# tskare/gpuaudiobench

Measured on AMD Instinct MI355X. Metric: audio_buffers_per_sec, higher is better.
Workload: dtype f32

## Files before the change

### gpuaudiobench_amd/csrc/k_conv_accel.hip

```cpp
#include <hip/hip_runtime.h>
#include <hip/hip_ext.h>

#include <cmath>
#include <cstdlib>
#include <algorithm>
#include <chrono>
#include <mutex>
#include <string>
#include <thread>
#include <type_traits>
#include <utility>
#include <vector>

#include "gab_common.hpp"
#include "gab_fft.hpp"
#include "k_conv_fdl.hpp"

namespace gab {
namespace fft {

void build_twiddles(float* t) {
    for (int m = 0; m < kTwiddleN; ++m) {
        double a = -2.0 * M_PI * (double)m / (double)kTwiddleN;
        t[2 * m] = (float)std::cos(a);
        t[2 * m + 1] = (float)std::sin(a);
    }
}

const cf* device_twiddles() {
    static std::mutex mu;
    static std::vector<cf*> per_device(64, nullptr);
    int dev = 0;
    GAB_HIP_CHECK(hipGetDevice(&dev));
    std::lock_guard<std::mutex> lock(mu);
    if (dev >= (int)per_device.size()) per_device.resize(dev + 1, nullptr);
    if (!per_device[dev]) {
        std::vector<float> host(2 * kTwiddleN);
        build_twiddles(host.data());
        cf* d = nullptr;
        GAB_HIP_CHECK(hipMalloc(&d, sizeof(cf) * kTwiddleN));
        GAB_HIP_CHECK(hipMemcpy(d, host.data(), sizeof(cf) * kTwiddleN, hipMemcpyHostToDevice));
        per_device[dev] = d;
    }
    return per_device[dev];
}

}

using fft::cf;
using fft::mk;

namespace {

constexpr int kB = 512;
constexpr int kNA = 1024;
constexpr int kNB = 4096;
constexpr int kSlots = 8;
constexpr int kBinsA = kNA / 2 + 1;
constexpr int kBinsB = kNB / 2 + 1;
constexpr int kThreads = 256;

using PadB = fft::Pad<16>;
constexpr int kLdsHalf = PadB::size(kNB);

using fft::partner_exchange;

template <int N, int R>
__device__ __forceinline__ void load_spectra(float4 (&c)[R], const float4* __restrict__ pm, int tid) {
    constexpr int NT = N / R;
#pragma unroll
    for (int r = 0; r < R; ++r) {
        const int k = tid + r * NT;
        if (r < R / 2) c[r] = pm[k];
        else if (r > R / 2) c[r] = pm[N - k];
        else c[r] = pm[tid == 0 ? k : N - k];
    }
}

template <int N, int R>
__device__ __forceinline__ void spectral_product(cf (&z)[R], const cf (&zraw)[R], const float4 (&c)[R],
                                                 int tid) {
#pragma unroll
    for (int r = 0; r < R; ++r) {
        cf P = mk(c[r].x, c[r].y), M = mk(c[r].z, c[r].w);
        if (r > R / 2 || (r == R / 2 && tid != 0)) {
            z[r] = fft::cfma_cjcj(zraw[r], M, fft::cmulc(z[r], P));
        } else {
            z[r] = fft::cfma_cj(zraw[r], M, fft::cmul(z[r], P));
        }
    }
}

template <bool STREAM, bool TAIL, bool LOOPED = false>
__device__ __forceinline__ void conv_one_buffer(
    const float* __restrict__ in, float* __restrict__ out, float* __restrict__ hist,
    const float4* __restrict__ pmA, const float4* __restrict__ pmB,
    const cf* __restrict__ tw, int T, int head, cf* __restrict__ lds) {
    cf* const lds0 = lds;
    cf* const lds1 = lds + kLdsHalf;
// ... 500 lines not shown
    unsigned* const gw = rt.counters + 32 * g;
    if (tid == 0) {
        const unsigned old = __hip_atomic_fetch_add(&gw[0], 1u, __ATOMIC_RELAXED, __HIP_MEMORY_SCOPE_AGENT);
        int role = 1;
        if (old + 1u == rt.epoch * (unsigned)members) {
            role = 2;
            __hip_atomic_store(&gw[1], 0u, __ATOMIC_RELAXED, __HIP_MEMORY_SCOPE_AGENT);
            asm volatile("s_waitcnt vmcnt(0)" ::: "memory");
            __hip_atomic_store(&gw[2], rt.epoch, __ATOMIC_RELAXED, __HIP_MEMORY_SCOPE_AGENT);
        } else {
            int tries = 0;
            while (__hip_atomic_load(&gw[2], __ATOMIC_RELAXED, __HIP_MEMORY_SCOPE_AGENT) != rt.epoch) {
                if (++tries > (1 << 10)) { role = 0; break; }
                __builtin_amdgcn_s_sleep(3);
            }
        }
        s_word = role;
    }
    __syncthreads();
    const int role = s_word;
    if (role == 0) return;
    const int row_f4 = members / 2;
    const auto srd = __builtin_amdgcn_make_buffer_rsrc(rt.park, 0, (int)((size_t)T * kB * 4), 0x00020000);
    const int col0 = 2 * first;
    unsigned drained = 0;
    for (;;) {
        __syncthreads();
        if (tid == 0) s_word = (int)__hip_atomic_fetch_add(&gw[1], 1u, __ATOMIC_RELAXED, __HIP_MEMORY_SCOPE_AGENT);
        __syncthreads();
        const int share = s_word;
        if (share >= members) break;
        const int i = share * kThreads + tid;
        const int sidx = i / row_f4, c = i - sidx * row_f4;
        const auto raw = __builtin_amdgcn_raw_buffer_load_b128(srd, 4u * (unsigned)(T * sidx + col0 + 4 * c), 0, 16);
        typedef float f4v __attribute__((ext_vector_type(4)));
        const f4v val = {__uint_as_float(raw[0]), __uint_as_float(raw[1]), __uint_as_float(raw[2]), __uint_as_float(raw[3])};
        float* const dst = rt.h_out + (size_t)T * sidx + col0 + 4 * c;
        asm volatile("global_store_dwordx4 %0, %1, off sc0 sc1" ::"v"(dst), "v"(val) : "memory");
        ++drained;
        if (role != 2) break;
    }
    asm volatile("s_waitcnt vmcnt(0)" ::: "memory");
    __syncthreads();
    GAB_RT_STAMP_MAX(g, 3);
    if (tid == 0 && drained) {
        const unsigned old = __hip_atomic_fetch_add(&rt.counters[32 * rt.groups], drained, __ATOMIC_RELAXED, __HIP_MEMORY_SCOPE_AGENT);
        if (old + drained == rt.epoch * (unsigned)gridDim.x) {
            __hip_atomic_store(rt.done, rt.epoch, __ATOMIC_RELAXED, __HIP_MEMORY_SCOPE_SYSTEM);
            GAB_RT_STAMP_MAX(64, 0);
        }
    }
}

__global__ __launch_bounds__(kThreads, 2) void conv_batch_kernel(
    const float* __restrict__ in, float* __restrict__ out, float* __restrict__ hist,
    const float4* __restrict__ pmA, const float4* __restrict__ pmB,
    const cf* __restrict__ tw, int T, int head, int n_buffers) {
    __shared__ cf lds[2 * kLdsHalf];
    const size_t step = (size_t)T * kB;
    for (int nb = 0; nb < n_buffers; ++nb)
        conv_one_buffer<true, true, true>(in + nb * step, out + nb * step, hist, pmA, pmB, tw, T,
                                             (head + nb) & (kSlots - 1), lds);
}

constexpr int kBatchBarriers = 6;

struct ConvEngine {
    const unsigned* doorbell;
    unsigned* relay;
    unsigned* progress;
    unsigned* completed;
    unsigned* error;
    int ring;
    int poll_every_period;
    unsigned* started;
    unsigned* resident;
    unsigned long long idle_ticks;
};
constexpr double kEngineIdleSeconds = 4.0;

typedef unsigned u4 __attribute__((ext_vector_type(4)));

constexpr int kB12Threads = 768;
constexpr int kB12SpecCf = 4 * kBinsA * 2;
constexpr int kB12Tw1Cf = 16 * 15;
constexpr int kB12Lds = 6 * kWaveImg + 2 * kLdsHalf + kB12SpecCf + kB12Tw1Cf;

template <int N, int R, int R0, int R1, class PM>
__device__ __forceinline__ void load_spectra_part(float4 (&c)[R1 - R0], PM pm, int tid) {
    constexpr int NT = N / R;
#pragma unroll
    for (int r = R0; r < R1; ++r) {
        const int k = tid + r * NT;
        if (r < R / 2) c[r - R0] = pm[k];
        else if (r > R / 2) c[r - R0] = pm[N - k];
        else c[r - R0] = pm[tid == 0 ? k : N - k];
    }
}
template <int N, int R, int R0, int R1>
__device__ __forceinline__ void spectral_product_part(cf (&z)[R], const cf (&zraw)[R1 - R0], const float4 (&c)[R1 - R0], int tid) {
#pragma unroll
    for (int r = R0; r < R1; ++r) {
        cf P = mk(c[r - R0].x, c[r - R0].y), M = mk(c[r - R0].z, c[r - R0].w);
        if (r > R / 2 || (r == R / 2 && tid != 0)) z[r] = fft::cfma_cjcj(zraw[r - R0], M, fft::cmulc(z[r], P));
        else z[r] = fft::cfma_cj(zraw[r - R0], M, fft::cmul(z[r], P));
    }
}

#ifdef GAB_ABLATE
__device__ unsigned long long g_split_stamps[2 * 8 * 8192];
#define GAB_B12BAR(period, i)                                                                                         \
    do {                                                                                                              \
        if ((sp.debug & 64) && ((period) == 32 || (period) == 33) && lane == 0)                                       \
            g_split_stamps[(((size_t)blockIdx.x * 12 + w) * 2 + ((period) - 32)) * 6 + (i)] = __builtin_amdgcn_s_memrealtime(); \
        __syncthreads();                                                                                              \
    } while (0)
#else
#define GAB_B12BAR(period, i) __syncthreads()
#endif
__device__ __forceinline__ void conv_split_batch12_resident(
    const float* __restrict__ in, float* __restrict__ out, float* __restrict__ hist,
    const float4* __restrict__ pmA, const ConvSplit& sp, const cf* __restrict__ tw, int T, int head0, int n_buffers,
    cf* __restrict__ lds) {
    cf* const far_img = lds + 6 * kWaveImg;
    float4* const spec = reinterpret_cast<float4*>(far_img + 2 * kLdsHalf);
    cf* const tw1 = reinterpret_cast<cf*>(spec + 4 * kBinsA);
    const int tid = threadIdx.x;
    const int d = xcd_contiguous(blockIdx.x, gridDim.x);
    const size_t step = (size_t)T * kB;
    {
        const float4* const gA = pmA + (size_t)(2 * d) * kBinsA;
        const float4* const gA2 = sp.pmA2 + (size_t)(2 * d) * kBinsA;
        for (int i = tid; i < 2 * kBinsA; i += kB12Threads) { spec[i] = gA[i]; spec[2 * kBinsA + i] = gA2[i]; }
        if (tid < 16) {
            cf pw[15];
            fft::powers_of<16>(tw[tid * (fft::kTwiddleN / 256)], pw);
#pragma unroll
            for (int r = 0; r < 15; ++r) tw1[tid * 15 + r] = pw[r];
        }
    }
    __syncthreads();
    const int lane = tid & 63;
    const int w = __builtin_amdgcn_readfirstlane(tid >> 6);
    const unsigned rb = (unsigned)lane + ((unsigned)lane >> 4);
    auto in_slot = [&](int slot) -> const float* { return in + (size_t)slot * step; };
    auto idle_period = [&]() { for (int i = 0; i < kBatchBarriers; ++i) __syncthreads(); };

    if (w >= 4) {
        const int g = __builtin_amdgcn_readfirstlane((w - 4) >> 2);
        const int ft = (tid - kThreads) & (kThreads - 1);
        cf* const img = far_img + g * kLdsHalf;
        const int q = 2 * d + g;
        const cf* const hp = reinterpret_cast<const cf*>(hist) + (size_t)q * kSlots * kB;
        cf* const cg = sp.carry + (size_t)q * kCarrySlots * kB;
        const size_t ca = (size_t)(2 * q) * kB, cb_ = ca + kB;
        const float4* const pf = sp.pmF + (size_t)q * kBinsB;
        using B16 = fft::Butterfly<16, false>;
        using B16i = fft::Butterfly<16, true>;
        cf tw2[15];
        fft::powers_of<16>(tw[ft], tw2);
        auto opaque_t = [&]() -> unsigned { unsigned v = (unsigned)ft; asm volatile("" : "+v"(v)); return v; };
        auto w0_of = [](unsigned t) -> unsigned { return t * 17u; };
        auto rd_of = [](unsigned t) -> unsigned { return t + (t >> 4); };
        auto w1_of = [](unsigned t) -> unsigned { const unsigned b1 = (t >> 4) * 256u + (t & 15u); return b1 + (b1 >> 4); };
        auto tw1row_of = [&](unsigned t) -> const cf* { return tw1 + (t & 15u) * 15u; };
        auto load_window = [&](auto part_tag, int nb, cf (&z)[16]) {
            constexpr int PART = decltype(part_tag)::value;
            const int head = (head0 + nb) & (kSlots - 1);
            int fo = ft;
            asm volatile("" : "+v"(fo));
            if constexpr (PART == 0) {
                const float* const cur = in_slot(nb);
                z[14] = mk(cur[ca + fo], cur[cb_ + fo]);
                z[15] = mk(cur[ca + fo + kThreads], cur[cb_ + fo + kThreads]);
            }
            constexpr int BL0 = PART == 0 ? 4 : 0, BL1 = PART == 0 ? 7 : 4;
            if (nb >= kSlots - 1) {
#pragma unroll
                for (int bl = BL0; bl < BL1; ++bl) {
                    const float* const src = in_slot(nb - (7 - bl));
                    z[2 * bl] = mk(src[ca + fo], src[cb_ + fo]);
                    z[2 * bl + 1] = mk(src[ca + fo + kThreads], src[cb_ + fo + kThreads]);
                }
            } else {
#pragma unroll
                for (int bl = BL0; bl < BL1; ++bl) {
                    if (nb - 7 + bl >= 0) {
                        const float* const src = in_slot(nb - (7 - bl));
                        z[2 * bl] = mk(src[ca + fo], src[cb_ + fo]);
                        z[2 * bl + 1] = mk(src[ca + fo + kThreads], src[cb_ + fo + kThreads]);
                    } else {
                        const int s = ((head + 1 + bl) & (kSlots - 1)) * kB;
                        z[2 * bl] = hp[s + fo];
                        z[2 * bl + 1] = hp[s + kThreads + fo];
                    }
                }
            }
        };
        cf z[16], zn[16];
        auto first_half = [&](int nb) {
#pragma unroll
            for (int r = 0; r < 16; ++r) z[r] = zn[r];
            B16::run(z);
            {
                const unsigned w0 = w0_of(opaque_t());
#pragma unroll
                for (int r = 0; r < 16; ++r) img[w0 + r] = z[B16::out_slot(r)];
            }
            GAB_B12BAR(nb, 0);
            {
                const unsigned t = opaque_t(), rd = rd_of(t);
                const cf* const tw1row = tw1row_of(t);
#pragma unroll
                for (int r = 0; r < 16; ++r) z[r] = img[rd + 272 * r];
#pragma unroll
                for (int r = 1; r < 16; ++r) z[r] = fft::cmul(z[r], tw1row[r - 1]);
            }
            B16::run(z);
            GAB_B12BAR(nb, 1);
            {
                const unsigned w1 = w1_of(opaque_t());
#pragma unroll
                for (int r = 0; r < 16; ++r) img[w1 + 17 * r] = z[B16::out_slot(r)];
            }
            __builtin_amdgcn_sched_barrier(0);
            float4 clo[8], chi[8];
            {
                int fo = ft;
                asm volatile("" : "+v"(fo));
                load_spectra_part<kNB, 16, 0, 8>(clo, pf, fo);
            }
            __builtin_amdgcn_sched_barrier(0);
            GAB_B12BAR(nb, 2);
            {
                const unsigned rd = rd_of(opaque_t());
#pragma unroll
                for (int r = 0; r < 16; ++r) z[r] = img[rd + 272 * r];
            }
#pragma unroll
            for (int r = 1; r < 16; ++r) z[r] = fft::cmul(z[r], tw2[r - 1]);
            __builtin_amdgcn_sched_barrier(0);
            {
                int fo = ft;
                asm volatile("" : "+v"(fo));
                load_spectra_part<kNB, 16, 8, 16>(chi, pf, fo);
            }
            __builtin_amdgcn_sched_barrier(0);
            B16::run(z);
            GAB_B12BAR(nb, 3);
            {
                const unsigned t = opaque_t();
#pragma unroll
                for (int r = 0; r < 16; ++r) img[t + 256u * r] = z[B16::out_slot(r)];
            }
            GAB_B12BAR(nb, 4);
            {
                cf o[16];
#pragma unroll
                for (int r = 0; r < 16; ++r) o[r] = z[B16::out_slot(r)];
#pragma unroll
                for (int r = 0; r < 16; ++r) z[r] = o[r];
                const unsigned t = opaque_t();
                const cf* const pb = img + (kNB - 256 * 15) - t;
                cf zp[8];
                zp[0] = img[(kNB - t) & (kNB - 1)];
#pragma unroll
                for (int r = 1; r < 8; ++r) zp[r] = pb[256 * (15 - r)];
                spectral_product_part<kNB, 16, 0, 8>(z, zp, clo, ft);
#pragma unroll
                for (int r = 0; r < 8; ++r) zp[r] = pb[256 * (7 - r)];
                spectral_product_part<kNB, 16, 8, 16>(z, zp, chi, ft);
            }
            B16i::run(z);
            GAB_B12BAR(nb, 5);
        };
        auto second_half = [&](int period, int nb_done, int nb_next) {
            if (nb_next >= 0) {
                load_window(std::integral_constant<int, 0>{}, nb_next, zn);
            } else {
#pragma unroll
                for (int r = 0; r < 16; ++r) zn[r] = mk(0.0f, 0.0f);
            }
            GAB_B12BAR(period, 0);
            if (nb_done >= 0) {
                const unsigned w0 = w0_of(opaque_t());
#pragma unroll
                for (int r = 0; r < 16; ++r) img[w0 + r] = z[B16i::out_slot(r)];
            }
            GAB_B12BAR(period, 1);
            if (nb_done >= 0) {
                const unsigned t = opaque_t(), rd = rd_of(t);
                const cf* const tw1row = tw1row_of(t);
#pragma unroll
                for (int r = 0; r < 16; ++r) z[r] = img[rd + 272 * r];
#pragma unroll
                for (int r = 1; r < 16; ++r) z[r] = fft::cmulc(z[r], tw1row[r - 1]);
                B16i::run(z);
            }
            GAB_B12BAR(period, 2);
            if (nb_done >= 0) {
                const unsigned w1 = w1_of(opaque_t());
#pragma unroll
                for (int r = 0; r < 16; ++r) img[w1 + 17 * r] = z[B16i::out_slot(r)];
            }
            __builtin_amdgcn_sched_barrier(0);
            if (nb_next >= 0) load_window(std::integral_constant<int, 1>{}, nb_next, zn);
            __builtin_amdgcn_sched_barrier(0);
            GAB_B12BAR(period, 3);
            if (nb_done >= 0) {
                const unsigned rd = rd_of(opaque_t());
#pragma unroll
                for (int r = 0; r < 16; ++r) z[r] = img[rd + 272 * r];
#pragma unroll
                for (int r = 1; r < 16; ++r) z[r] = fft::cmulc(z[r], tw2[r - 1]);
                cf x12, x13, x14, x15;
                B16i::run_last4(z, x12, x13, x14, x15);
                const int head = (head0 + nb_done) & (kSlots - 1);
                cf* const c1 = cg + ((head + 1) & (kCarrySlots - 1)) * kB;
                cf* const c2 = cg + ((head + 2) & (kCarrySlots - 1)) * kB;
                c1[ft] = x12;
                c1[ft + kThreads] = x13;
                c2[ft] = x14;
                c2[ft + kThreads] = x15;
            }
            GAB_B12BAR(period, 4);
            if (nb_done >= 0) asm volatile("s_waitcnt vmcnt(0)" ::: "memory");
            GAB_B12BAR(period, 5);
        };
        const int first = (g - head0) & 1;
        int nb = 0;
        if (first == 1) {
            second_half(0, -1, 1 < n_buffers ? 1 : -1);
            nb = 1;
        } else if (n_buffers > 0) {
            load_window(std::integral_constant<int, 0>{}, 0, zn);
            load_window(std::integral_constant<int, 1>{}, 0, zn);
        }
        for (;;) {
            if (nb > n_buffers) break;
            if (nb < n_buffers) first_half(nb); else idle_period();
            ++nb;
            if (nb > n_buffers) break;
            second_half(nb, nb - 1 < n_buffers ? nb - 1 : -1, nb + 1 < n_buffers ? nb + 1 : -1);
            ++nb;
        }
    } else if (w < 2) {
        const int q = 2 * d + w;
        cf* const hp = reinterpret_cast<cf*>(hist) + (size_t)q * kSlots * kB;
        cf* const img = lds + w * kWaveImg;
        cf* const hand = lds + (2 + w) * kWaveImg;
        const float4* const sa = spec + w * kBinsA;
        const float4* const sa2 = spec + (2 + w) * kBinsA;
        using WF = fft::WaveFFT1024<false>;
        WF::Lean t;
        WF::load_twiddles(t, tw, lane);
        const size_t xoff = (size_t)(2 * q) * kB;
        cf z[16], prev[8], nxt[8];
        auto product_from_image = [&](cf (&v)[16], const float4* sp_lds) {
            {
                cf zp[8];
                float4 ch[8];
#pragma unroll
                for (int r = 0; r < 8; ++r) zp[r] = img[PadA16::at((kNA - (lane + 64 * r)) & (kNA - 1))];
                load_spectra_part<kNA, 16, 0, 8>(ch, sp_lds, lane);
                spectral_product_part<kNA, 16, 0, 8>(v, zp, ch, lane);
            }
            __builtin_amdgcn_sched_barrier(0);
            {
                cf zp[8];
                float4 ch[8];
#pragma unroll
                for (int r = 0; r < 8; ++r) zp[r] = img[PadA16::at((kNA - (lane + 64 * (8 + r))) & (kNA - 1))];
                load_spectra_part<kNA, 16, 8, 16>(ch, sp_lds, lane);
                spectral_product_part<kNA, 16, 8, 16>(v, zp, ch, lane);
            }
        };
        {
            const int s1 = ((head0 + kSlots - 1) & (kSlots - 1)) * kB, s2 = ((head0 + kSlots - 2) & (kSlots - 1)) * kB;
#pragma unroll
            for (int j = 0; j < 8; ++j) z[j] = hp[s2 + lane + 64 * j];
#pragma unroll
            for (int j = 0; j < 8; ++j) prev[j] = hp[s1 + lane + 64 * j];
            if (n_buffers > 0) {
                const float* const x0 = in_slot(0) + xoff;
#pragma unroll
                for (int j = 0; j < 8; ++j) nxt[j] = mk(x0[lane + 64 * j], x0[kB + lane + 64 * j]);
            }
#pragma unroll
            for (int j = 0; j < 8; ++j) z[8 + j] = prev[j];
            WF::run(z, img, t, lane, WF::NoHook());
#pragma unroll
            for (int r = 0; r < 16; ++r) img[rb + 68 * r] = z[r];
            __builtin_amdgcn_wave_barrier();
        }
        for (int nb = 0; nb < n_buffers; ++nb) {
            const int head = (head0 + nb) & (kSlots - 1);
            {
                cf share[16];
#pragma unroll
                for (int r = 0; r < 16; ++r) share[r] = img[rb + 68 * r];
                product_from_image(share, sa2);
                GAB_B12BAR(nb, 0);
#pragma unroll
                for (int r = 0; r < 16; ++r) hand[rb + 68 * r] = share[r];
            }
            __builtin_amdgcn_sched_barrier(0);
#pragma unroll
            for (int j = 0; j < 8; ++j) { z[j] = prev[j]; z[8 + j] = nxt[j]; }
            if (nb + kSlots >= n_buffers) {
#pragma unroll
                for (int j = 0; j < 8; ++j) hp[head * kB + lane + 64 * j] = nxt[j];
            }
#pragma unroll
            for (int j = 0; j < 8; ++j) prev[j] = nxt[j];
            if (nb + 1 < n_buffers) {
                int lo = lane;
                asm volatile("" : "+v"(lo));
                const float* const xa = in_slot(nb + 1) + xoff + lo;
#pragma unroll
                for (int j = 0; j < 8; ++j) nxt[j] = mk(xa[64 * j], xa[kB + 64 * j]);
            }
            WF::run(z, img, t, lane, [&](int i) { GAB_B12BAR(nb, 1 + i); });
            GAB_B12BAR(nb, 3);
#pragma unroll
            for (int r = 0; r < 16; ++r) img[rb + 68 * r] = z[r];
            __builtin_amdgcn_wave_barrier();
            product_from_image(z, sa);
            GAB_B12BAR(nb, 4);
#pragma unroll
            for (int r = 0; r < 16; ++r) hand[rb + 68 * r] = fft::cadd(z[r], hand[rb + 68 * r]);
            GAB_B12BAR(nb, 5);
        }
        idle_period();
    } else {
        const int pr = w - 2;
        const cf* const hand = lds + (2 + pr) * kWaveImg;
        cf* const img = lds + (4 + pr) * kWaveImg;
        const cf* const other = lds + (4 + (1 - pr)) * kWaveImg;
        const cf* const cg = sp.carry + (size_t)(2 * d + pr) * kCarrySlots * kB;
        using WFi = fft::WaveFFT1024<true>;
        WFi::Lean t;
        WFi::load_twiddles(t, tw, lane);
        idle_period();
        for (int nb = 1; nb <= n_buffers; ++nb) {
            const int b = nb - 1;
            const int head = (head0 + b) & (kSlots - 1);
            float* const outb = out + (size_t)b * step;
            cf z[16], y[8], park[8];
#pragma unroll
            for (int r = 0; r < 16; ++r) z[r] = hand[rb + 68 * r];
            {
                int lo = lane;
                asm volatile("" : "+v"(lo));
                const unsigned long long* const cy = reinterpret_cast<const unsigned long long*>(cg + (head & (kCarrySlots - 1)) * kB + lo);
#pragma unroll
                for (int j = 0; j < 8; ++j) {
                    const unsigned long long v = __hip_atomic_load(cy + 64 * j, __ATOMIC_RELAXED, __HIP_MEMORY_SCOPE_AGENT);
                    park[j] = mk(__uint_as_float((unsigned)v), __uint_as_float((unsigned)(v >> 32)));
                }
            }
            GAB_B12BAR(nb, 0);
            WFi::run(z, img, t, lane, [&](int i) { GAB_B12BAR(nb, 1 + i); });
#pragma unroll
            for (int j = 0; j < 8; ++j) y[j] = fft::cadd(z[8 + j], park[j]);
            GAB_B12BAR(nb, 3);
            if (pr == 0) {
#pragma unroll
                for (int j = 0; j < 4; ++j) img[lane + 64 * j] = y[4 + j];
            } else {
#pragma unroll
                for (int j = 0; j < 4; ++j) img[lane + 64 * j] = y[j];
            }
            GAB_B12BAR(nb, 4);
            {
                float* const o0 = outb + 4 * (size_t)d;
                if (pr == 0) {
#pragma unroll
                    for (int j = 0; j < 4; ++j) {
                        const cf theirs = other[lane + 64 * j];
                        *reinterpret_cast<float4*>(o0 + (size_t)T * (lane + 64 * j)) = make_float4(y[j].x, y[j].y, theirs.x, theirs.y);
                    }
                } else {
#pragma unroll
                    for (int j = 0; j < 4; ++j) {
                        const cf theirs = other[lane + 64 * j];
                        *reinterpret_cast<float4*>(o0 + (size_t)T * (lane + 64 * (4 + j))) = make_float4(theirs.x, theirs.y, y[4 + j].x, y[4 + j].y);
                    }
                }
            }
            GAB_B12BAR(nb, 5);
        }
    }
}

__global__ __launch_bounds__(kB12Threads) void conv_split_batch12_kernel(
    const float* __restrict__ in, float* __restrict__ out, float* __restrict__ hist,
    const float4* __restrict__ pmA, ConvSplit sp, const cf* __restrict__ tw, int T, int head0, int n_buffers) {
    __shared__ __attribute__((aligned(16))) cf lds[kB12Lds];
    conv_split_batch12_resident(in, out, hist, pmA, sp, tw, T, head0, n_buffers, lds);
}

#ifdef GAB_ABLATE
#define GAB_E12BAR(i)                                                                                                 \
    do {                                                                                                              \
        if ((sp.debug & 64) && (nb == 4000 || nb == 4001) && lane == 0)                                               \
            g_split_stamps[(((size_t)blockIdx.x * 12 + w) * 2 + (nb - 4000)) * 6 + (i)] = __builtin_amdgcn_s_memrealtime(); \
        __syncthreads();                                                                                              \
    } while (0)
#else
#define GAB_E12BAR(i) __syncthreads()
#endif
__device__ __forceinline__ void conv_split_engine12_resident(
    const float* __restrict__ in, float* __restrict__ out, float* __restrict__ hist,
    const float4* __restrict__ pmA, const ConvSplit& sp, const cf* __restrict__ tw, int T, int head0,
    const ConvEngine& eng, cf* __restrict__ lds, unsigned* __restrict__ s_door) {
    constexpr bool ENGINE = true;
    constexpr int n_buffers = 0;
    (void)ENGINE; (void)n_buffers;
    cf* const far_img = lds + 6 * kWaveImg;
    float4* const spec = reinterpret_cast<float4*>(far_img + 2 * kLdsHalf);
    cf* const tw1 = reinterpret_cast<cf*>(spec + 4 * kBinsA);
    const int tid = threadIdx.x;
    const int d = xcd_contiguous(blockIdx.x, gridDim.x);
    const size_t step = (size_t)T * kB;
    {
        const float4* const gA = pmA + (size_t)(2 * d) * kBinsA;
        const float4* const gA2 = sp.pmA2 + (size_t)(2 * d) * kBinsA;
        for (int i = tid; i < 2 * kBinsA; i += kB12Threads) { spec[i] = gA[i]; spec[2 * kBinsA + i] = gA2[i]; }
        if (tid < 16) {
            cf pw[15];
            fft::powers_of<16>(tw[tid * (fft::kTwiddleN / 256)], pw);
#pragma unroll
            for (int r = 0; r < 15; ++r) tw1[tid * 15 + r] = pw[r];
        }
    }
    constexpr int kPoller = 2 * 64;
    auto read_door = [&]() -> unsigned {
        if (blockIdx.x == 0) {
            const unsigned v = __hip_atomic_load(eng.doorbell, __ATOMIC_RELAXED, __HIP_MEMORY_SCOPE_SYSTEM);
            __hip_atomic_store(eng.relay, v, __ATOMIC_RELAXED, __HIP_MEMORY_SCOPE_AGENT);
            return v;
        }
        return __hip_atomic_load(eng.relay, __ATOMIC_RELAXED, __HIP_MEMORY_SCOPE_AGENT);
    };
    if (tid == 0) {
        s_door[2] = 0;
        const unsigned before = __hip_atomic_fetch_add(eng.started, 1u, __ATOMIC_RELAXED, __HIP_MEMORY_SCOPE_AGENT);
        if (before == 0) __hip_atomic_store(&eng.resident[0], 1u, __ATOMIC_RELAXED, __HIP_MEMORY_SCOPE_SYSTEM);
        if (before + 1 == gridDim.x) __hip_atomic_store(&eng.resident[1], gridDim.x, __ATOMIC_RELAXED, __HIP_MEMORY_SCOPE_SYSTEM);
    }
    __syncthreads();
    const int lane = tid & 63;
    const int w = __builtin_amdgcn_readfirstlane(tid >> 6);
    const unsigned rb = (unsigned)lane + ((unsigned)lane >> 4);
    const bool aggregator = blockIdx.x == (gridDim.x > 1 ? 1u : 0u);
    unsigned reported = 0;
    auto aggregate_request = [&](u4& a, u4& b) {
        const auto srd = __builtin_amdgcn_make_buffer_rsrc(eng.progress, 0, (int)(8u * gridDim.x), 0x00020000);
        a = __builtin_amdgcn_raw_buffer_load_b128(srd, 32u * (unsigned)lane, 0, 16);
        b = __builtin_amdgcn_raw_buffer_load_b128(srd, 32u * (unsigned)lane + 16u, 0, 16);
    };
    auto aggregate_report = [&](const u4& a, const u4& b) {
        const unsigned words = 2u * gridDim.x;
        auto pick = [&](unsigned v, unsigned idx) { return idx < words ? v : 0xffffffffu; };
        unsigned m = min(min(min(pick(a[0], 8u * lane), pick(a[1], 8u * lane + 1)), min(pick(a[2], 8u * lane + 2), pick(a[3], 8u * lane + 3))),
                         min(min(pick(b[0], 8u * lane + 4), pick(b[1], 8u * lane + 5)), min(pick(b[2], 8u * lane + 6), pick(b[3], 8u * lane + 7))));
#pragma unroll
        for (int o = 32; o > 0; o >>= 1) m = min(m, (unsigned)__shfl_xor((int)m, o));
        if (m != reported) {
            reported = m;
            if (lane == 0) __hip_atomic_store(eng.completed, m, __ATOMIC_RELAXED, __HIP_MEMORY_SCOPE_SYSTEM);
        }
    };
    auto gate = [&](int nb, bool idle) -> int {
        {
            if (idle && __builtin_amdgcn_readfirstlane(s_door[2]) != 0) return -1;
            bool look = !idle;
            for (;;) {
                if (look) {
                    const unsigned D = __builtin_amdgcn_readfirstlane(s_door[nb & 1]);
                    const int pub = (int)(D & 0x3fffffffu);
                    const bool stop = (D >> 31) != 0, flush = ((D >> 30) & 1u) != 0;
                    if (pub >= nb + 2 || ((stop || flush) && pub >= nb + 1)) return pub;
                    if (stop) return -1;
                }
                look = true;
                __syncthreads();
                if (w == 2) {
                    unsigned v = 0;
                    int tries = 0;
                    const unsigned long long t_poll = __builtin_amdgcn_s_memrealtime();
                    for (;;) {
                        u4 pa, pb;
                        if (aggregator) aggregate_request(pa, pb);
                        unsigned mine = 0;
                        if (lane == 0) mine = read_door();
                        v = __builtin_amdgcn_readfirstlane(mine);
                        if (aggregator) aggregate_report(pa, pb);
                        const int p2 = (int)(v & 0x3fffffffu);
                        if (p2 >= nb + 2 || (v >> 31) || (((v >> 30) & 1u) && p2 >= nb + 1)) break;
                        if ((++tries & 255) == 0 && __builtin_amdgcn_s_memrealtime() - t_poll > eng.idle_ticks) {
                            if (lane == 0) {
                                __hip_atomic_store(eng.error, 1u, __ATOMIC_RELAXED, __HIP_MEMORY_SCOPE_SYSTEM);
                                s_door[2] = 1;
                            }
                            v = 0x80000000u | (unsigned)(p2 < nb ? p2 : nb);
                            break;
                        }
                        __builtin_amdgcn_s_sleep(6);
                    }
                    if (lane == 0) s_door[nb & 1] = v;
                }
                __syncthreads();
            }
        }
    };
    auto in_slot = [&](int slot) -> const float* { return in + (size_t)slot * step; };
    auto next_slot = [&](int slot) -> int { return (ENGINE && slot + 1 == eng.ring) ? 0 : slot + 1; };
    auto ld = [](const float* p) -> float {
        if constexpr (ENGINE)
            return __hip_atomic_load(p, __ATOMIC_RELAXED, __HIP_MEMORY_SCOPE_SYSTEM);
        else return *p;
    };

    auto idle_period = [&]() { for (int i = 0; i < kBatchBarriers; ++i) __syncthreads(); };

    if (w >= 4) {
        const int g = __builtin_amdgcn_readfirstlane((w - 4) >> 2);
        const int ft = (tid - kThreads) & (kThreads - 1);
        cf* const img = far_img + g * kLdsHalf;
        const int q = 2 * d + g;
        const cf* const hp = reinterpret_cast<const cf*>(hist) + (size_t)q * kSlots * kB;
        cf* const cg = sp.carry + (size_t)q * kCarrySlots * kB;
        const size_t ca = (size_t)(2 * q) * kB, cb_ = ca + kB;
        const float4* const pf = sp.pmF + (size_t)q * kBinsB;
        using B16 = fft::Butterfly<16, false>;
        using B16i = fft::Butterfly<16, true>;
        const cf tw2_base = tw[ft];
        auto tw2_of = [&](cf (&w)[15]) {
            cf b = tw2_base;
            asm volatile("" : "+v"(b.x), "+v"(b.y));
            fft::powers_of<16>(b, w);
        };
        auto opaque_t = [&]() -> unsigned { unsigned v = (unsigned)ft; asm volatile("" : "+v"(v)); return v; };
        auto w0_of = [](unsigned t) -> unsigned { return t * 17u; };
        auto rd_of = [](unsigned t) -> unsigned { return t + (t >> 4); };
        auto w1_of = [](unsigned t) -> unsigned { const unsigned b1 = (t >> 4) * 256u + (t & 15u); return b1 + (b1 >> 4); };
        auto tw1row_of = [&](unsigned t) -> const cf* { return tw1 + (t & 15u) * 15u; };
        auto load_window = [&](auto part_tag, auto first_tag, int nb, int slot, int slot_before, cf (&z)[16]) {
            constexpr int PART = decltype(part_tag)::value;
            constexpr bool FIRST = decltype(first_tag)::value;
            const int head = (head0 + nb) & (kSlots - 1);
            int fo = ft;
            asm volatile("" : "+v"(fo));
            if constexpr (PART == 0) {
                const float* const cur = in_slot(slot);
                z[14] = mk(ld(cur + ca + fo), ld(cur + cb_ + fo));
                z[15] = mk(ld(cur + ca + fo + kThreads), ld(cur + cb_ + fo + kThreads));
                if constexpr (!FIRST) {
                    const float* const prv = in_slot(slot_before);
                    z[12] = mk(ld(prv + ca + fo), ld(prv + cb_ + fo));
                    z[13] = mk(ld(prv + ca + fo + kThreads), ld(prv + cb_ + fo + kThreads));
                } else {
                    const int s6 = ((head + kSlots - 1) & (kSlots - 1)) * kB;
                    z[12] = hp[s6 + fo];
                    z[13] = hp[s6 + kThreads + fo];
                }
#pragma unroll
                for (int bl = 4; bl < 6; ++bl) {
                    const int sb = ((head + 1 + bl) & (kSlots - 1)) * kB;
                    z[2 * bl] = hp[sb + fo];
                    z[2 * bl + 1] = hp[sb + kThreads + fo];
                }
            } else {
#pragma unroll
                for (int bl = 0; bl < 4; ++bl) {
                    const int sb = ((head + 1 + bl) & (kSlots - 1)) * kB;
                    z[2 * bl] = hp[sb + fo];
                    z[2 * bl + 1] = hp[sb + kThreads + fo];
                }
            }
        };
        cf z[16], zn[16];
        auto first_half = [&](int nb) {
#pragma unroll
            for (int r = 0; r < 16; ++r) z[r] = zn[r];
            B16::run(z);
            {
                const unsigned w0 = w0_of(opaque_t());
#pragma unroll
                for (int r = 0; r < 16; ++r) img[w0 + r] = z[B16::out_slot(r)];
            }
            GAB_E12BAR(0);
            {
                const unsigned t = opaque_t(), rd = rd_of(t);
                const cf* const tw1row = tw1row_of(t);
#pragma unroll
                for (int r = 0; r < 16; ++r) z[r] = img[rd + 272 * r];
#pragma unroll
                for (int r = 1; r < 16; ++r) z[r] = fft::cmul(z[r], tw1row[r - 1]);
            }
            B16::run(z);
            GAB_E12BAR(1);
            {
                const unsigned w1 = w1_of(opaque_t());
#pragma unroll
                for (int r = 0; r < 16; ++r) img[w1 + 17 * r] = z[B16::out_slot(r)];
            }
            __builtin_amdgcn_sched_barrier(0);
            float4 clo[8], chi[8];
            {
                int fo = ft;
                asm volatile("" : "+v"(fo));
                load_spectra_part<kNB, 16, 0, 8>(clo, pf, fo);
            }
            __builtin_amdgcn_sched_barrier(0);
            GAB_E12BAR(2);
            {
                const unsigned rd = rd_of(opaque_t());
#pragma unroll
                for (int r = 0; r < 16; ++r) z[r] = img[rd + 272 * r];
            }
            {
                cf tw2[15];
                tw2_of(tw2);
#pragma unroll
                for (int r = 1; r < 16; ++r) z[r] = fft::cmul(z[r], tw2[r - 1]);
            }
            __builtin_amdgcn_sched_barrier(0);
            {
                int fo = ft;
                asm volatile("" : "+v"(fo));
                load_spectra_part<kNB, 16, 8, 16>(chi, pf, fo);
            }
            __builtin_amdgcn_sched_barrier(0);
            B16::run(z);
            GAB_E12BAR(3);
            {
                const unsigned t = opaque_t();
#pragma unroll
                for (int r = 0; r < 16; ++r) img[t + 256u * r] = z[B16::out_slot(r)];
            }
            GAB_E12BAR(4);
            {
                cf o[16];
#pragma unroll
                for (int r = 0; r < 16; ++r) o[r] = z[B16::out_slot(r)];
#pragma unroll
                for (int r = 0; r < 16; ++r) z[r] = o[r];
                const unsigned t = opaque_t();
                const cf* const pb = img + (kNB - 256 * 15) - t;
                cf zp[8];
                zp[0] = img[(kNB - t) & (kNB - 1)];
#pragma unroll
                for (int r = 1; r < 8; ++r) zp[r] = pb[256 * (15 - r)];
                spectral_product_part<kNB, 16, 0, 8>(z, zp, clo, ft);
#pragma unroll
                for (int r = 0; r < 8; ++r) zp[r] = pb[256 * (7 - r)];
                spectral_product_part<kNB, 16, 8, 16>(z, zp, chi, ft);
            }
            B16i::run(z);
            GAB_E12BAR(5);
        };
        auto second_half = [&](int period, int nb_done, int nb_next, int slot_next, int slot_now) {
            const int nb = period;
            (void)nb;
            if (nb_next >= 0) {
                load_window(std::integral_constant<int, 0>{}, std::false_type{}, nb_next, slot_next, slot_now, zn);
            } else {
#pragma unroll
                for (int r = 0; r < 16; ++r) zn[r] = mk(0.0f, 0.0f);
            }
            GAB_E12BAR(0);
            if (nb_done >= 0) {
                const unsigned w0 = w0_of(opaque_t());
#pragma unroll
                for (int r = 0; r < 16; ++r) img[w0 + r] = z[B16i::out_slot(r)];
            }
            GAB_E12BAR(1);
            if (nb_done >= 0) {
                const unsigned t = opaque_t(), rd = rd_of(t);
                const cf* const tw1row = tw1row_of(t);
#pragma unroll
                for (int r = 0; r < 16; ++r) z[r] = img[rd + 272 * r];
#pragma unroll
                for (int r = 1; r < 16; ++r) z[r] = fft::cmulc(z[r], tw1row[r - 1]);
                B16i::run(z);
            }
            GAB_E12BAR(2);
            if (nb_done >= 0) {
                const unsigned w1 = w1_of(opaque_t());
#pragma unroll
                for (int r = 0; r < 16; ++r) img[w1 + 17 * r] = z[B16i::out_slot(r)];
            }
            __builtin_amdgcn_sched_barrier(0);
            if (nb_next >= 0) load_window(std::integral_constant<int, 1>{}, std::false_type{}, nb_next, slot_next, slot_now, zn);
            __builtin_amdgcn_sched_barrier(0);
            GAB_E12BAR(3);
            if (nb_done >= 0) {
                const unsigned rd = rd_of(opaque_t());
#pragma unroll
                for (int r = 0; r < 16; ++r) z[r] = img[rd + 272 * r];
                {
                    cf tw2[15];
                    tw2_of(tw2);
#pragma unroll
                    for (int r = 1; r < 16; ++r) z[r] = fft::cmulc(z[r], tw2[r - 1]);
                }
                cf x12, x13, x14, x15;
                B16i::run_last4(z, x12, x13, x14, x15);
                const int head = (head0 + nb_done) & (kSlots - 1);
                cf* const c1 = cg + ((head + 1) & (kCarrySlots - 1)) * kB;
                cf* const c2 = cg + ((head + 2) & (kCarrySlots - 1)) * kB;
                c1[ft] = x12;
                c1[ft + kThreads] = x13;
                c2[ft] = x14;
                c2[ft + kThreads] = x15;
            }
            GAB_E12BAR(4);
            if (nb_done >= 0) asm volatile("s_waitcnt vmcnt(0)" ::: "memory");
            GAB_E12BAR(5);
        };
        bool in_flight = false, have_window = false;
        int nb = 0, slot = 0;
        for (;;) {
            int avail = gate(nb, true);
            if (nb >= avail) break;
            for (;;) {
                const bool mine = ((head0 + nb) & 1) == g;
                if (mine) {
                    if (!have_window) {
                        load_window(std::integral_constant<int, 0>{}, std::true_type{}, nb, slot, 0, zn);
                        load_window(std::integral_constant<int, 1>{}, std::true_type{}, nb, slot, 0, zn);
                    }
                    first_half(nb);
                    in_flight = true;
                    have_window = false;
                } else {
                    const bool can = nb + 1 < avail;
                    second_half(nb, in_flight ? nb - 1 : -1, can ? nb + 1 : -1, next_slot(slot), slot);
                    have_window = can;
                    in_flight = false;
// ... 1573 lines not shown
```

Baseline: 207,500.

## Exchange far-FFT conjugate partner bins via permlane32 swap instead of LDS

Remaps the far-segment thread-to-column assignment so that each lane's conjugate-mirror column sits in the opposite half of the same wave. The spectral product can then fetch partner bins with permlane32_swap instead of writing the whole FFT image to LDS and reading it back. Columns 0 and 128 get special handling in wave 0. This removes an LDS store/load round trip per period, but the two barrier calls are kept, and the change adds cross-lane permute instructions and a remapping that has to be correct.

```diff
diff --git a/gpuaudiobench_amd/csrc/k_conv_accel.hip b/gpuaudiobench_amd/csrc/k_conv_accel.hip
--- a/gpuaudiobench_amd/csrc/k_conv_accel.hip
+++ b/gpuaudiobench_amd/csrc/k_conv_accel.hip
@@ -696,13 +696,71 @@
         else c[r - R0] = pm[tid == 0 ? k : N - k];
     }
 }
+template <int R>
+__device__ __forceinline__ void spectral_product_bin(cf& z, cf zraw, float4 c, int r, int tid) {
+    cf P = mk(c.x, c.y), M = mk(c.z, c.w);
+    if (r > R / 2 || (r == R / 2 && tid != 0)) z = fft::cfma_cjcj(zraw, M, fft::cmulc(z, P));
+    else z = fft::cfma_cj(zraw, M, fft::cmul(z, P));
+}
 template <int N, int R, int R0, int R1>
 __device__ __forceinline__ void spectral_product_part(cf (&z)[R], const cf (&zraw)[R1 - R0], const float4 (&c)[R1 - R0], int tid) {
 #pragma unroll
-    for (int r = R0; r < R1; ++r) {
-        cf P = mk(c[r - R0].x, c[r - R0].y), M = mk(c[r - R0].z, c[r - R0].w);
-        if (r > R / 2 || (r == R / 2 && tid != 0)) z[r] = fft::cfma_cjcj(zraw[r - R0], M, fft::cmulc(z[r], P));
-        else z[r] = fft::cfma_cj(zraw[r - R0], M, fft::cmul(z[r], P));
+    for (int r = R0; r < R1; ++r) spectral_product_bin<R>(z[r], zraw[r - R0], c[r - R0], r, tid);
+}
+
+__device__ __forceinline__ int far_column(int fw, int lane) {
+    const int c = lane < 32 ? 32 * fw + lane : 256 - 32 * fw - (lane - 32);
+    return c == 256 ? 128 : c;
+}
+__device__ __forceinline__ void half_swap(float& u, float& v) {
+    const auto a = __builtin_amdgcn_permlane32_swap(__float_as_uint(u), __float_as_uint(v), false, false);
+    const auto b = __builtin_amdgcn_permlane32_swap(a[1], a[0], false, false);
+    u = __uint_as_float(b[0]);
+    v = __uint_as_float(b[1]);
+}
+__device__ __forceinline__ void half_swap(cf& u, cf& v) {
+    float ux = u.x, uy = u.y, vx = v.x, vy = v.y;
+    half_swap(ux, vx);
+    half_swap(uy, vy);
+    u = mk(ux, uy);
+    v = mk(vx, vy);
+}
+__device__ __forceinline__ void far_partner_product(cf (&z)[16], const float4 (&clo)[8], const float4 (&chi)[8],
+                                                    int col, bool wave0, int lane) {
+    constexpr int G = 2;
+    cf raw[16];
+#pragma unroll
+    for (int r = 0; r < 16; ++r) raw[r] = z[r];
+#pragma unroll
+    for (int h = 0; h < 8 / G; ++h) {
+        cf pa[G], pb[G];
+#pragma unroll
+        for (int j = 0; j < G; ++j) {
+            const int r = G * h + j;
+            pa[j] = raw[15 - r];
+            pb[j] = raw[r];
+            half_swap(pa[j], pb[j]);
+        }
+        if (wave0) {
+            asm volatile("" ::: "memory");
+            if ((lane & 31) == 0) {
+                asm volatile("" ::: "memory");
+                const bool c0 = lane == 0;
+#pragma unroll
+                for (int j = 0; j < G; ++j) {
+                    const int r = G * h + j;
+                    pa[j] = c0 ? raw[(16 - r) & 15] : raw[15 - r];
+                    pb[j] = c0 ? raw[(r + 1) & 15] : raw[r];
+                }
+            }
+        }
+#pragma unroll
+        for (int j = 0; j < G; ++j) {
+            const int r = G * h + j;
+            spectral_product_bin<16>(z[r], pa[j], clo[r], r, col);
+            spectral_product_bin<16>(z[15 - r], pb[j], chi[7 - r], 15 - r, col);
+        }
+        __builtin_amdgcn_sched_barrier(0);
     }
 }
 
@@ -747,7 +805,8 @@
 
     if (w >= 4) {
         const int g = __builtin_amdgcn_readfirstlane((w - 4) >> 2);
-        const int ft = (tid - kThreads) & (kThreads - 1);
+        const bool fw0 = ((w - 4) & 3) == 0;
+        const int ft = far_column((w - 4) & 3, lane);
         cf* const img = far_img + g * kLdsHalf;
         const int q = 2 * d + g;
         const cf* const hp = reinterpret_cast<const cf*>(hist) + (size_t)q * kSlots * kB;
@@ -847,11 +906,6 @@
             __builtin_amdgcn_sched_barrier(0);
             B16::run(z);
             GAB_B12BAR(nb, 3);
-            {
-                const unsigned t = opaque_t();
-#pragma unroll
-                for (int r = 0; r < 16; ++r) img[t + 256u * r] = z[B16::out_slot(r)];
-            }
             GAB_B12BAR(nb, 4);
             {
                 cf o[16];
@@ -859,16 +913,7 @@
                 for (int r = 0; r < 16; ++r) o[r] = z[B16::out_slot(r)];
 #pragma unroll
                 for (int r = 0; r < 16; ++r) z[r] = o[r];
-                const unsigned t = opaque_t();
-                const cf* const pb = img + (kNB - 256 * 15) - t;
-                cf zp[8];
-                zp[0] = img[(kNB - t) & (kNB - 1)];
-#pragma unroll
-                for (int r = 1; r < 8; ++r) zp[r] = pb[256 * (15 - r)];
-                spectral_product_part<kNB, 16, 0, 8>(z, zp, clo, ft);
-#pragma unroll
-                for (int r = 0; r < 8; ++r) zp[r] = pb[256 * (7 - r)];
-                spectral_product_part<kNB, 16, 8, 16>(z, zp, chi, ft);
+                far_partner_product(z, clo, chi, ft, fw0, lane);
             }
             B16i::run(z);
             GAB_B12BAR(nb, 5);
@@ -1226,7 +1271,8 @@
 
     if (w >= 4) {
         const int g = __builtin_amdgcn_readfirstlane((w - 4) >> 2);
-        const int ft = (tid - kThreads) & (kThreads - 1);
+        const bool fw0 = ((w - 4) & 3) == 0;
+        const int ft = far_column((w - 4) & 3, lane);
         cf* const img = far_img + g * kLdsHalf;
         const int q = 2 * d + g;
         const cf* const hp = reinterpret_cast<const cf*>(hist) + (size_t)q * kSlots * kB;
@@ -1335,11 +1381,6 @@
             __builtin_amdgcn_sched_barrier(0);
             B16::run(z);
             GAB_E12BAR(3);
-            {
-                const unsigned t = opaque_t();
-#pragma unroll
-                for (int r = 0; r < 16; ++r) img[t + 256u * r] = z[B16::out_slot(r)];
-            }
             GAB_E12BAR(4);
             {
                 cf o[16];
@@ -1347,16 +1388,7 @@
                 for (int r = 0; r < 16; ++r) o[r] = z[B16::out_slot(r)];
 #pragma unroll
                 for (int r = 0; r < 16; ++r) z[r] = o[r];
-                const unsigned t = opaque_t();
-                const cf* const pb = img + (kNB - 256 * 15) - t;
-                cf zp[8];
-                zp[0] = img[(kNB - t) & (kNB - 1)];
-#pragma unroll
-                for (int r = 1; r < 8; ++r) zp[r] = pb[256 * (15 - r)];
-                spectral_product_part<kNB, 16, 0, 8>(z, zp, clo, ft);
-#pragma unroll
-                for (int r = 0; r < 8; ++r) zp[r] = pb[256 * (7 - r)];
-                spectral_product_part<kNB, 16, 8, 16>(z, zp, chi, ft);
+                far_partner_product(z, clo, chi, ft, fw0, lane);
             }
             B16i::run(z);
             GAB_E12BAR(5);
```

New measurement: 204,500. 1.5% lower.

## Restructure far-partition FFT LDS layout to cut per-period barriers from six to four

Applied to the files above, without the earlier changes.

Introduces a new LDS index layout for the far-tail 4096-point FFT in which the forward, spectral-product and inverse stages read and write each thread's values in place. This removes the separate write-back/read barrier pairs between passes. All wave roles in the batch12 kernel are re-synchronized to four barriers per period instead of six. The aim is less block-wide synchronization stall per audio buffer, at the cost of more intricate index arithmetic, a side slot for the Nyquist partner, and a higher risk of LDS bank conflicts or indexing errors.

```diff
diff --git a/gpuaudiobench_amd/csrc/k_conv_accel.hip b/gpuaudiobench_amd/csrc/k_conv_accel.hip
--- a/gpuaudiobench_amd/csrc/k_conv_accel.hip
+++ b/gpuaudiobench_amd/csrc/k_conv_accel.hip
@@ -15,6 +15,7 @@
 #include "gab_common.hpp"
 #include "gab_fft.hpp"
 #include "k_conv_fdl.hpp"
+#include "k_conv_far_layout.hpp"
 
 namespace gab {
 namespace fft {
@@ -681,6 +682,7 @@
 typedef unsigned u4 __attribute__((ext_vector_type(4)));
 
 constexpr int kB12Threads = 768;
+constexpr int kB12Barriers = 4;
 constexpr int kB12SpecCf = 4 * kBinsA * 2;
 constexpr int kB12Tw1Cf = 16 * 15;
 constexpr int kB12Lds = 6 * kWaveImg + 2 * kLdsHalf + kB12SpecCf + kB12Tw1Cf;
@@ -711,7 +713,7 @@
 #define GAB_B12BAR(period, i)                                                                                         \
     do {                                                                                                              \
         if ((sp.debug & 64) && ((period) == 32 || (period) == 33) && lane == 0)                                       \
-            g_split_stamps[(((size_t)blockIdx.x * 12 + w) * 2 + ((period) - 32)) * 6 + (i)] = __builtin_amdgcn_s_memrealtime(); \
+            g_split_stamps[(((size_t)blockIdx.x * 12 + w) * 2 + ((period) - 32)) * kB12Barriers + (i)] = __builtin_amdgcn_s_memrealtime(); \
         __syncthreads();                                                                                              \
     } while (0)
 #else
@@ -743,7 +745,7 @@
     const int w = __builtin_amdgcn_readfirstlane(tid >> 6);
     const unsigned rb = (unsigned)lane + ((unsigned)lane >> 4);
     auto in_slot = [&](int slot) -> const float* { return in + (size_t)slot * step; };
-    auto idle_period = [&]() { for (int i = 0; i < kBatchBarriers; ++i) __syncthreads(); };
+    auto idle_period = [&]() { for (int i = 0; i < kB12Barriers; ++i) __syncthreads(); };
 
     if (w >= 4) {
         const int g = __builtin_amdgcn_readfirstlane((w - 4) >> 2);
@@ -758,10 +760,8 @@
         using B16i = fft::Butterfly<16, true>;
         cf tw2[15];
         fft::powers_of<16>(tw[ft], tw2);
+        namespace FL = far_layout;
         auto opaque_t = [&]() -> unsigned { unsigned v = (unsigned)ft; asm volatile("" : "+v"(v)); return v; };
-        auto w0_of = [](unsigned t) -> unsigned { return t * 17u; };
-        auto rd_of = [](unsigned t) -> unsigned { return t + (t >> 4); };
-        auto w1_of = [](unsigned t) -> unsigned { const unsigned b1 = (t >> 4) * 256u + (t & 15u); return b1 + (b1 >> 4); };
         auto tw1row_of = [&](unsigned t) -> const cf* { return tw1 + (t & 15u) * 15u; };
         auto load_window = [&](auto part_tag, int nb, cf (&z)[16]) {
             constexpr int PART = decltype(part_tag)::value;
@@ -797,47 +797,58 @@
             }
         };
         cf z[16], zn[16];
-        auto first_half = [&](int nb) {
+        float4 clo[8], chi[8];
+        auto step_pass0 = [&]() {
 #pragma unroll
             for (int r = 0; r < 16; ++r) z[r] = zn[r];
             B16::run(z);
+            const unsigned t = opaque_t();
+#pragma unroll
+            for (int r = 0; r < 16; ++r) img[FL::pass0_write(t, r)] = z[B16::out_slot(r)];
+        };
+        auto step_pass1 = [&]() {
             {
-                const unsigned w0 = w0_of(opaque_t());
-#pragma unroll
-                for (int r = 0; r < 16; ++r) img[w0 + r] = z[B16::out_slot(r)];
-            }
-            GAB_B12BAR(nb, 0);
+                const unsigned t = opaque_t(), a = FL::a_base(t);
+                const cf* const tw1row = tw1row_of(t);
+#pragma unroll
+                for (int r = 0; r < 16; ++r) z[r] = img[a + 272 * r];
+#pragma unroll
+                for (int r = 1; r < 16; ++r) z[r] = fft::cmul(z[r], tw1row[r - 1]);
+            }
+            B16::run(z);
+            __builtin_amdgcn_sched_barrier(0);
             {
-                const unsigned t = opaque_t(), rd = rd_of(t);
-                const cf* const tw1row = tw1row_of(t);
-#pragma unroll
-                for (int r = 0; r < 16; ++r) z[r] = img[rd + 272 * r];
-#pragma unroll
-                for (int r = 1; r < 16; ++r) z[r] = fft::cmul(z[r], tw1row[r - 1]);
-            }
-            B16::run(z);
-            GAB_B12BAR(nb, 1);
-            {
-                const unsigned w1 = w1_of(opaque_t());
-#pragma unroll
-                for (int r = 0; r < 16; ++r) img[w1 + 17 * r] = z[B16::out_slot(r)];
+                const unsigned a = FL::a_base(opaque_t());
+#pragma unroll
+                for (int r = 0; r < 16; ++r) img[a + 272 * r] = z[B16::out_slot(r)];
             }
             __builtin_amdgcn_sched_barrier(0);
-            float4 clo[8], chi[8];
             {
                 int fo = ft;
                 asm volatile("" : "+v"(fo));
                 load_spectra_part<kNB, 16, 0, 8>(clo, pf, fo);
             }
             __builtin_amdgcn_sched_barrier(0);
-            GAB_B12BAR(nb, 2);
+        };
+        auto step_pass2 = [&]() {
             {
-                const unsigned rd = rd_of(opaque_t());
-#pragma unroll
-                for (int r = 0; r < 16; ++r) z[r] = img[rd + 272 * r];
+                const unsigned b = FL::pass2_base(opaque_t());
+#pragma unroll
+                for (int r = 0; r < 16; ++r) z[r] = img[b + 17 * r];
             }
 #pragma unroll
             for (int r = 1; r < 16; ++r) z[r] = fft::cmul(z[r], tw2[r - 1]);
+            B16::run(z);
+            __builtin_amdgcn_sched_barrier(0);
+            {
+                const unsigned t = opaque_t(), b = FL::pass2_base(t);
+#pragma unroll
+                for (int r = 0; r < 16; ++r) img[b + 17 * r] = z[B16::out_slot(r)];
+                if (t == 0) {
+#pragma unroll
+                    for (int r = 0; r < 16; ++r) img[FL::side_slot(r)] = z[B16::out_slot(r)];
+                }
+            }
             __builtin_amdgcn_sched_barrier(0);
             {
                 int fo = ft;
@@ -845,33 +856,78 @@
                 load_spectra_part<kNB, 16, 8, 16>(chi, pf, fo);
             }
             __builtin_amdgcn_sched_barrier(0);
-            B16::run(z);
-            GAB_B12BAR(nb, 3);
-            {
-                const unsigned t = opaque_t();
-#pragma unroll
-                for (int r = 0; r < 16; ++r) img[t + 256u * r] = z[B16::out_slot(r)];
-            }
-            GAB_B12BAR(nb, 4);
+        };
+        auto step_partner = [&]() {
             {
                 cf o[16];
 #pragma unroll
                 for (int r = 0; r < 16; ++r) o[r] = z[B16::out_slot(r)];
 #pragma unroll
                 for (int r = 0; r < 16; ++r) z[r] = o[r];
-                const unsigned t = opaque_t();
-                const cf* const pb = img + (kNB - 256 * 15) - t;
+                const cf* const pb = img + FL::partner_base(opaque_t());
                 cf zp[8];
-                zp[0] = img[(kNB - t) & (kNB - 1)];
-#pragma unroll
-                for (int r = 1; r < 8; ++r) zp[r] = pb[256 * (15 - r)];
+#pragma unroll
+                for (int r = 0; r < 8; ++r) zp[r] = pb[17 * (15 - r)];
                 spectral_product_part<kNB, 16, 0, 8>(z, zp, clo, ft);
 #pragma unroll
-                for (int r = 0; r < 8; ++r) zp[r] = pb[256 * (7 - r)];
+                for (int r = 0; r < 8; ++r) zp[r] = pb[17 * (7 - r)];
                 spectral_product_part<kNB, 16, 8, 16>(z, zp, chi, ft);
             }
             B16i::run(z);
-            GAB_B12BAR(nb, 5);
+            __builtin_amdgcn_sched_barrier(0);
+            {
+                cf* const pb = img + FL::partner_base(opaque_t());
+#pragma unroll
+                for (int r = 0; r < 16; ++r) pb[17 * r] = z[B16i::out_slot(r)];
+            }
+        };
+        auto step_inv1 = [&]() {
+            {
+                const unsigned t = opaque_t(), p0 = FL::inv1_first(t), pb = FL::inv1_base(t);
+                const cf* const tw1row = tw1row_of(t);
+                z[0] = img[p0];
+#pragma unroll
+                for (int r = 1; r < 16; ++r) z[r] = img[pb - 272 * r];
+#pragma unroll
+                for (int r = 1; r < 16; ++r) z[r] = fft::cmulc(z[r], tw1row[r - 1]);
+            }
+            B16i::run(z);
+            __builtin_amdgcn_sched_barrier(0);
+            {
+                const unsigned t = opaque_t(), p0 = FL::inv1_first(t), pb = FL::inv1_base(t);
+                img[p0] = z[B16i::out_slot(0)];
+#pragma unroll
+                for (int r = 1; r < 16; ++r) img[pb - 272 * r] = z[B16i::out_slot(r)];
+            }
+        };
+        auto step_inv2 = [&](int nb_done) {
+            {
+                const unsigned t = opaque_t(), p0 = FL::inv2_first(t), pb = FL::inv2_base(t);
+                z[0] = img[p0];
+#pragma unroll
+                for (int r = 1; r < 16; ++r) z[r] = img[pb - r];
+            }
+#pragma unroll
+            for (int r = 1; r < 16; ++r) z[r] = fft::cmulc(z[r], tw2[r - 1]);
+            cf x12, x13, x14, x15;
+            B16i::run_last4(z, x12, x13, x14, x15);
+            const int head = (head0 + nb_done) & (kSlots - 1);
+            cf* const c1 = cg + ((head + 1) & (kCarrySlots - 1)) * kB;
+            cf* const c2 = cg + ((head + 2) & (kCarrySlots - 1)) * kB;
+            c1[ft] = x12;
+            c1[ft + kThreads] = x13;
+            c2[ft] = x14;
+            c2[ft + kThreads] = x15;
+        };
+        auto first_half = [&](int nb) {
+            step_pass0();
+            GAB_B12BAR(nb, 0);
+            step_pass1();
+            GAB_B12BAR(nb, 1);
+            step_pass2();
+            GAB_B12BAR(nb, 2);
+            step_partner();
+            GAB_B12BAR(nb, 3);
         };
         auto second_half = [&](int period, int nb_done, int nb_next) {
             if (nb_next >= 0) {
@@ -880,51 +936,15 @@
 #pragma unroll
                 for (int r = 0; r < 16; ++r) zn[r] = mk(0.0f, 0.0f);
             }
+            __builtin_amdgcn_sched_barrier(0);
+            if (nb_done >= 0) step_inv1();
             GAB_B12BAR(period, 0);
-            if (nb_done >= 0) {
-                const unsigned w0 = w0_of(opaque_t());
-#pragma unroll
-                for (int r = 0; r < 16; ++r) img[w0 + r] = z[B16i::out_slot(r)];
-            }
+            if (nb_done >= 0) step_inv2(nb_done);
             GAB_B12BAR(period, 1);
-            if (nb_done >= 0) {
-                const unsigned t = opaque_t(), rd = rd_of(t);
-                const cf* const tw1row = tw1row_of(t);
-#pragma unroll
-                for (int r = 0; r < 16; ++r) z[r] = img[rd + 272 * r];
-#pragma unroll
-                for (int r = 1; r < 16; ++r) z[r] = fft::cmulc(z[r], tw1row[r - 1]);
-                B16i::run(z);
-            }
+            if (nb_next >= 0) load_window(std::integral_constant<int, 1>{}, nb_next, zn);
             GAB_B12BAR(period, 2);
-            if (nb_done >= 0) {
-                const unsigned w1 = w1_of(opaque_t());
-#pragma unroll
-                for (int r = 0; r < 16; ++r) img[w1 + 17 * r] = z[B16i::out_slot(r)];
-            }
-            __builtin_amdgcn_sched_barrier(0);
-            if (nb_next >= 0) load_window(std::integral_constant<int, 1>{}, nb_next, zn);
-            __builtin_amdgcn_sched_barrier(0);
+            if (nb_done >= 0) asm volatile("s_waitcnt vmcnt(0)" ::: "memory");
             GAB_B12BAR(period, 3);
-            if (nb_done >= 0) {
-                const unsigned rd = rd_of(opaque_t());
-#pragma unroll
-                for (int r = 0; r < 16; ++r) z[r] = img[rd + 272 * r];
-#pragma unroll
-                for (int r = 1; r < 16; ++r) z[r] = fft::cmulc(z[r], tw2[r - 1]);
-                cf x12, x13, x14, x15;
-                B16i::run_last4(z, x12, x13, x14, x15);
-                const int head = (head0 + nb_done) & (kSlots - 1);
-                cf* const c1 = cg + ((head + 1) & (kCarrySlots - 1)) * kB;
-                cf* const c2 = cg + ((head + 2) & (kCarrySlots - 1)) * kB;
-                c1[ft] = x12;
-                c1[ft + kThreads] = x13;
-                c2[ft] = x14;
-                c2[ft + kThreads] = x15;
-            }
-            GAB_B12BAR(period, 4);
-            if (nb_done >= 0) asm volatile("s_waitcnt vmcnt(0)" ::: "memory");
-            GAB_B12BAR(period, 5);
         };
         const int first = (g - head0) & 1;
         int nb = 0;
@@ -1019,16 +1039,15 @@
 #pragma unroll
                 for (int j = 0; j < 8; ++j) nxt[j] = mk(xa[64 * j], xa[kB + 64 * j]);
             }
-            WF::run(z, img, t, lane, [&](int i) { GAB_B12BAR(nb, 1 + i); });
-            GAB_B12BAR(nb, 3);
+            WF::run(z, img, t, lane, [&](int i) { if (i == 1) GAB_B12BAR(nb, 1); else __builtin_amdgcn_sched_barrier(0); });
+            GAB_B12BAR(nb, 2);
 #pragma unroll
             for (int r = 0; r < 16; ++r) img[rb + 68 * r] = z[r];
             __builtin_amdgcn_wave_barrier();
             product_from_image(z, sa);
-            GAB_B12BAR(nb, 4);
 #pragma unroll
             for (int r = 0; r < 16; ++r) hand[rb + 68 * r] = fft::cadd(z[r], hand[rb + 68 * r]);
-            GAB_B12BAR(nb, 5);
+            GAB_B12BAR(nb, 3);
         }
         idle_period();
     } else {
@@ -1059,10 +1078,9 @@
                 }
             }
             GAB_B12BAR(nb, 0);
-            WFi::run(z, img, t, lane, [&](int i) { GAB_B12BAR(nb, 1 + i); });
+            WFi::run(z, img, t, lane, [&](int i) { if (i == 1) GAB_B12BAR(nb, 1); else __builtin_amdgcn_sched_barrier(0); });
 #pragma unroll
             for (int j = 0; j < 8; ++j) y[j] = fft::cadd(z[8 + j], park[j]);
-            GAB_B12BAR(nb, 3);
             if (pr == 0) {
 #pragma unroll
                 for (int j = 0; j < 4; ++j) img[lane + 64 * j] = y[4 + j];
@@ -1070,7 +1088,7 @@
 #pragma unroll
                 for (int j = 0; j < 4; ++j) img[lane + 64 * j] = y[j];
             }
-            GAB_B12BAR(nb, 4);
+            GAB_B12BAR(nb, 2);
             {
                 float* const o0 = outb + 4 * (size_t)d;
                 if (pr == 0) {
@@ -1087,7 +1105,7 @@
                     }
                 }
             }
-            GAB_B12BAR(nb, 5);
+            GAB_B12BAR(nb, 3);
         }
     }
 }
diff --git a/gpuaudiobench_amd/csrc/k_conv_far_layout.hpp b/gpuaudiobench_amd/csrc/k_conv_far_layout.hpp
--- /dev/null
+++ b/gpuaudiobench_amd/csrc/k_conv_far_layout.hpp
@@ -0,0 +1,43 @@
+#pragma once
+
+#if defined(__HIPCC__)
+#define GAB_FAR_HD __host__ __device__
+#else
+#define GAB_FAR_HD
+#endif
+
+namespace gab {
+namespace far_layout {
+
+constexpr unsigned kN = 4096;
+constexpr unsigned kThreads = 256;
+constexpr unsigned kImage = kN + (kN >> 4);
+constexpr unsigned kSide = 17 * 16 + 16;
+
+GAB_FAR_HD constexpr unsigned a_base(unsigned t) { return t + (t >> 4); }
+GAB_FAR_HD constexpr unsigned b_base(unsigned u) { return u == kThreads ? kSide : (u & 15u) + 272u * (u >> 4); }
+
+GAB_FAR_HD constexpr unsigned pass0_write(unsigned t, unsigned r) { return 17u * t + r; }
+GAB_FAR_HD constexpr unsigned pass1_slot(unsigned t, unsigned r) { return a_base(t) + 272u * r; }
+GAB_FAR_HD constexpr unsigned pass2_slot(unsigned t, unsigned r) { return b_base(t) + 17u * r; }
+GAB_FAR_HD constexpr unsigned side_slot(unsigned r) { return kSide + 17u * ((r + 15u) & 15u); }
+GAB_FAR_HD constexpr unsigned partner_read(unsigned t, unsigned r) { return b_base(kThreads - t) + 17u * (15u - r); }
+GAB_FAR_HD constexpr unsigned inv0_write(unsigned t, unsigned r) { return b_base(kThreads - t) + 17u * r; }
+GAB_FAR_HD constexpr unsigned inv1_slot(unsigned v, unsigned s) {
+    return b_base(kThreads - (v >> 4) - 16u * s) + 17u * (v & 15u);
+}
+GAB_FAR_HD constexpr unsigned inv2_slot(unsigned u, unsigned r) {
+    return b_base(kThreads - r - 16u * (u >> 4)) + 17u * (u & 15u);
+}
+
+GAB_FAR_HD constexpr unsigned pass2_base(unsigned t) { return (t & 15u) + 272u * (t >> 4); }
+GAB_FAR_HD constexpr unsigned partner_base(unsigned t) { return b_base(kThreads - t); }
+GAB_FAR_HD constexpr unsigned inv1_base(unsigned v) {
+    return ((v >> 4) == 0 ? kImage : kN - (v >> 4)) + 17u * (v & 15u);
+}
+GAB_FAR_HD constexpr unsigned inv1_first(unsigned v) { return (v >> 4) == 0 ? kSide + 17u * (v & 15u) : inv1_base(v); }
+GAB_FAR_HD constexpr unsigned inv2_base(unsigned u) { return 16u + 272u * (15u - (u >> 4)) + 17u * (u & 15u); }
+GAB_FAR_HD constexpr unsigned inv2_first(unsigned u) { return (u >> 4) == 0 ? kSide + 17u * (u & 15u) : inv2_base(u) + 256u; }
+
+}
+}
```

Measured after the change: 200,400 before, 201,500 after, median of 6. About the same (+0.5%).
